# zhuye98/ICL

Measured on AMD Instinct MI355X. Metric: 3D volumes/sec/node (fwd+bwd, 96^3 patch), higher is better.
Workload: dtype f32; 1 GPU; 3D U-Net ICL BraTS-shape synthetic 96x96x96, num_classes=2, batch=2 per GPU (1 labeled + 1 unlabeled), full ICL step incl. SGD; global_batch=2, parallelism=dp1, launch=hipGraph replay

## Files before the change

### icl_amd/_lib.py

```python
from __future__ import annotations

import ctypes
import os
from ctypes import c_char_p, c_double, c_float, c_int, c_int64, c_void_p

import torch

_HERE = os.path.dirname(os.path.abspath(__file__))
DEFAULT_LIB = os.path.join(_HERE, "libicl_hip.so")

_lib = None
_lib_path = None
_host_pointers_ok = False

P, I, L, F = c_void_p, c_int, c_int64, c_float
D = c_double

_SIGNATURES = {
    "icl_abi_version": (c_int, []),
    "icl_last_error": (c_char_p, []),
    "icl_last_kernel_name": (c_char_p, []),
    "icl_conv3d_packed_elems": (c_int64, [I, I, I, I]),
    "icl_conv3d_pack_weights": (c_int, [P, P, I, I, I, I, P]),
    "icl_conv3d_pack_weights_both": (c_int, [P, P, P, I, I, I, P]),
# ... 2 lines not shown
    "icl_conv3d_fwd": (c_int, [P, P, P, P, P, I, I, I, I, I, I, I, L, L, P]),
    "icl_scalar_combine": (c_int, [P, P, I, I, P, P]),
    "icl_conv3d_split_ws_bytes": (c_int64, [I, I]),
    "icl_conv3d_split_weights_multi": (c_int, [P, P, P, P, I, P]),
    "icl_conv3d_fwd_presplit": (c_int, [P, P, P, P, I, I, I, I, I, I, L, L, P]),
    "icl_conv3d_fwd_presplit_ws_bytes": (c_int64, [I, I, I, I, I, I]),
    "icl_conv3d_fwd_presplit_ws": (c_int, [P, P, P, P, P, I, I, I, I, I, I, L, L, P]),
    "icl_conv3d_fwd_stats_slots": (c_int, [I, I, I, I, I, I]),
    "icl_conv3d_fwd_presplit_stats": (c_int, [P, P, P, P, P, I, I, I, I, I, I, L, L, P]),
    "icl_norm_fwd_given_stats": (c_int, [P, P, P, P, P, P, P, P, P, I, I, L, I, I, F, F, P, I, P]),
    "icl_conv3d_wgrad_ws_bytes": (c_int64, [I, I, I, I]),
    "icl_conv3d_wgrad": (c_int, [P, P, P, P, P, I, I, I, I, I, I, I, L, L, P]),
    "icl_conv3d_wgrad_slabs": (c_int, [P, P, P, I, I, I, I, I, I, I, L, L, P, P]),
    "icl_conv3d_wgrad_reduce_multi": (c_int, [P, P, P, P, P, P, I, P]),
    "icl_norm_ws_bytes": (c_int64, [I, I, L]),
    "icl_norm_fwd": (c_int, [P, P, P, P, P, P, P, P, I, I, L, I, I, I, F, F, P, P]),
    "icl_norm_bwd": (c_int, [P, P, P, P, P, P, P, P, P, I, I, L, I, I, I, P, P]),
    "icl_norm_res_fwd": (c_int, [P, P, P, P, P, P, P, P, P, I, I, L, I, I, I, F, F, P, P]),
    "icl_norm_res_bwd": (c_int, [P, P, P, P, P, P, P, P, P, P, P, I, I, L, I, I, I, P, P]),
    "icl_rstd_from_var": (c_int, [P, P, I, F, P]),
    "icl_norm_finalize_stats": (c_int, [P, I, I, I, F, P, P, P, P]),
    "icl_norm_apply": (c_int, [P, P, P, I, I, L, P]),
    "icl_maxpool2_fwd_norm": (c_int, [P, P, P, P, L, I, I, I, I, P]),
    "icl_upsample2x_concat_norm": (c_int, [P, P, P, P, P, I, I, I, I, I, I, P]),
    "icl_conv1x1_dropout_norm": (c_int, [P, P, P, P, P, I, I, I, L, I, I, ctypes.c_uint32, F, P, P]),
    "icl_conv1x1_wgrad_dropout_norm": (c_int, [P, P, P, P, P, P, I, I, I, L, L, ctypes.c_uint32, F, P, P]),
    "icl_maxpool2_fwd": (c_int, [P, P, P, L, I, I, I, I, P]),
    "icl_maxpool2_bwd": (c_int, [P, P, P, L, I, I, I, I, P]),
    "icl_maxpool2_bwd_add": (c_int, [P, P, P, P, I, I, I, I, I, I, L, P]),
    "icl_trilinear_fwd": (c_int, [P, P, I, I, I, I, I, I, I, I, L, I, P]),
    "icl_trilinear_bwd_ws_bytes": (c_int64, [I, I, I, I, I, I, I, I]),
    "icl_trilinear_bwd": (c_int, [P, P, P, I, I, I, I, I, I, I, I, L, I, P]),
    "icl_copy_rows": (c_int, [P, P, L, L, L, L, P]),
    "icl_concat2": (c_int, [P, L, P, L, P, P]),
    "icl_dwconv3_fwd": (c_int, [P, P, P, I, I, I, I, I, I, P]),
    "icl_dwconv3_wgrad_ws_bytes": (c_int64, [I, I, I, I, I]),
    "icl_dwconv3_wgrad": (c_int, [P, P, P, P, I, I, I, I, I, P]),
    "icl_conv1x1_small": (c_int, [P, P, P, P, I, I, I, L, I, I, P]),
    "icl_conv1x1_dropout": (c_int, [P, P, P, P, I, I, I, L, I, I, I, ctypes.c_uint32, F, P, P]),
    "icl_conv1x1_wgrad_dropout": (c_int, [P, P, P, P, P, I, I, I, L, L, ctypes.c_uint32, F, P, P]),
    "icl_dropout": (c_int, [P, P, L, ctypes.c_uint32, F, P, P]),
    "icl_drop_path": (c_int, [P, P, L, L, ctypes.c_uint32, F, P, P]),
    "icl_drop_path_add": (c_int, [P, P, P, L, L, ctypes.c_uint32, F, P, P]),
    "icl_loss_fwd": (c_int, [P, P, P, P, P, P, I, I, L, I, I, P]),
    "icl_window_attn_bias_elems": (c_int64, [I, I]),
    "icl_depth_to_space2": (c_int, [P, P, I, I, I, I, I, L, P]),
    "icl_space_to_depth2": (c_int, [P, P, I, I, I, I, I, L, P]),
    "icl_colsum_multi": (c_int, [P, P, P, P, I, P]),
    "icl_gather_rows": (c_int, [P, P, P, L, L, L, I, P]),
    "icl_gather_rows_sum2": (c_int, [P, P, P, L, L, L, I, P]),
    "icl_im2col3": (c_int, [P, P, I, I, I, I, I, P]),
    "icl_im2col3_planes": (c_int, [P, P, I, I, I, I, I, P]),
    "icl_conv3d_cin1_fwd": (c_int, [P, P, P, P, I, I, I, I, I, L, L, P]),
    "icl_conv3d_cin1_wgrad_ws_bytes": (c_int64, [I, I, I]),
    "icl_conv3d_cin1_wgrad": (c_int, [P, P, P, P, I, I, I, I, I, L, L, P]),
    "icl_col2im3": (c_int, [P, P, I, I, I, I, I, P]),
    "icl_linear_ws_bytes": (c_int64, [L, I, I, I]),
    "icl_linear_fwd": (c_int, [P, P, P, P, P, L, I, I, I, P]),
    "icl_linear_dgrad": (c_int, [P, P, P, P, L, I, I, P]),
    "icl_linear_bwd_small": (c_int, [P, P, P, P, P, P, L, I, I, P]),
    "icl_linear_wgrad_small": (c_int, [P, P, P, P, L, I, I, P]),
    "icl_linear_dgrad_sgd": (c_int, [P, P, P, P, P, P, L, I, I, F, F, F, I, P, P]),
    "icl_gemm_ws_bytes": (c_int64, [L, I, I, I]),
    "icl_gemm": (c_int, [P, P, P, P, P, L, I, I, L, L, L, I, I, I, I, L, L, L, P]),
    "icl_linear_wgrad_ws_bytes": (c_int64, [L, I, I]),
    "icl_linear_wgrad": (c_int, [P, P, P, P, P, L, I, I, P]),
    "icl_conv1x1_wgrad_ws_bytes": (c_int64, [I, L, I, I]),
    "icl_conv1x1_wgrad": (c_int, [P, P, P, P, P, I, I, I, L, L, L, P]),
    "icl_relpos_bias_fwd": (c_int, [P, P, P, I, I, I, P]),
    "icl_window_attn_fwd": (c_int, [P, P, P, P, P, I, I, I, I, I, F, P]),
    "icl_window_attn_bwd": (c_int, [P, P, P, P, P, P, P, P, I, I, I, I, I, F, P]),
    "icl_window_attn_bwd_chunks": (c_int, [I, I, I, I, I]),
    "icl_window_attn_fwd_drop": (c_int, [P, P, P, P, P, I, I, I, I, I, F, ctypes.c_uint32, F, P, P]),
    "icl_window_attn_keep_probe": (c_int, [P, c_int64, I, ctypes.c_uint32, F, P, P]),
    "icl_window_attn_bwd_drop": (c_int, [P, P, P, P, P, P, P, P, I, I, I, I, I, F, ctypes.c_uint32, F, P, P]),
    "icl_relpos_bias_bwd_sum": (c_int, [P, I, P, P, P, L, I, I, P]),
    "icl_layernorm_fwd": (c_int, [P, P, P, P, P, P, L, I, F, P]),
    "icl_layernorm_bwd_ws_bytes": (c_int64, [L, I]),
    "icl_layernorm_bwd": (c_int, [P, P, P, P, P, P, P, P, P, L, I, P]),
    "icl_gelu_fwd": (c_int, [P, P, L, P]),
    "icl_gelu_bwd": (c_int, [P, P, P, L, P]),
    "icl_attn_fwd": (c_int, [P, P, P, P, P, I, I, I, I, I, F, P]),
    "icl_attn_bwd": (c_int, [P, P, P, P, P, P, P, P, P, I, I, I, I, I, F, P]),
    "icl_attn_bwd_ws_bytes": (c_int64, [I, I, I, I, I]),
    "icl_attn_bwd_ws": (c_int, [P, P, P, P, P, P, P, P, P, P, I, I, I, I, I, F, P]),
    "icl_crop_rotflip": (c_int, [P, P, P, I, P, P, I, I, I, P]),
    "icl_volume_feed": (c_int, [P, P, P, P, I, P, P, I, I, I, P]),
    "icl_slice_augment": (c_int, [P, P, P, P, I, P, P, I, I, P]),
    "icl_slice_resize": (c_int, [P, P, L, I, I, I, I, I, P]),
    "icl_sgd_step": (c_int, [P, P, P, L, F, F, F, I, P, P]),
    "icl_sgd_step_factored": (c_int, [P, P, P, P, I, I, I, F, F, F, I, P, P]),
    "icl_sgd_step_factored_narrow": (c_int, [P, P, P, P, I, I, I, F, F, F, I, P, I, P]),
    "icl_sgd_factored_split_ws_bytes": (c_int64, [I, I, I]),
    "icl_sgd_step_factored_split": (c_int, [P, P, P, P, P, I, I, I, F, F, F, I, P, P]),
    "icl_sgd_step_multi": (c_int, [P, P, P, P, I, F, F, F, I, P, P]),
    "icl_loss_bwd": (c_int, [P, P, P, P, P, P, P, P, I, I, L, I, I, P]),
    "icl_loss_fwd_multi": (c_int, [P, I, P]),
    "icl_loss_bwd_multi": (c_int, [P, I, P]),
    "icl_qchain_stage": (c_int, [P, P]),
    "icl_qchain_wgrad": (c_int, [P, P, P, P, P, P, P, P, I, P]),
    "icl_seg_metrics_ws_bytes": (c_int64, [I, I, I, I]),
    "icl_seg_metrics": (c_int, [P, I, P, I, I, I, I, I, I, P, P, P]),
    "icl_seg_surface_ws_bytes": (c_int64, [I, I, I, I]),
    "icl_seg_surface_metrics": (c_int, [P, I, P, I, I, I, I, I, D, D, D, D, P, P, P, P]),
    "icl_window_gather": (c_int, [P, P, P, I, I, I, I, I, I, I, I, I, I, I, I, I, I, P]),
    "icl_window_accumulate": (c_int, [P, P, P, P, P, I, I, I, I, I, I, I, I, I, P]),
# ... 49 lines not shown
```

### icl_amd/csrc/icl_abi.inc

```

#include "kernels/common.h"
#include "kernels/norm.h"
#include "kernels/pool_resize.h"
#include "kernels/reduce.h"
#include "kernels/conv_mfma.h"
#include "kernels/conv_mfma_static.h"
#include "kernels/conv_mfma_flat.h"
#include "kernels/conv_bf16x3.h"
#include "kernels/conv_bf16x3_ws.h"
#include "kernels/conv_wgrad_tr.h"
#include "kernels/conv_wgrad_zs.h"
#include "kernels/conv_cin1.h"
#include "kernels/misc.h"
#include "kernels/loss.h"
#include "kernels/optim.h"
#include "kernels/winattn.h"
#include "kernels/linear_wgrad.h"
#include "kernels/token.h"
#include "kernels/gemm.h"
#include "kernels/datafeed.h"
#include "kernels/qchain.h"
#include "kernels/metrics.h"
#include "kernels/metrics_surface.h"
#include "kernels/window.h"
// ... 1815 lines not shown
  } else {
    if (tiled) ICL_LAUNCH((icl::attn_bwd_kv_kernel<8, true>), g1, dim3(256), 0, st, q, kv, logits, stats, out, gout, glog, gkv, b, h, nc, n, scale, pq);
    else ICL_LAUNCH((icl::attn_bwd_kv_kernel<8, false>), g1, dim3(256), 0, st, q, kv, logits, stats, out, gout, glog, gkv, b, h, nc, n, scale, pq);
    if (!pq) ICL_LAUNCH((icl::attn_bwd_q_kernel<8, 256>), g2, dim3(256), 0, st, kv, logits, stats, out, gout, glog, gq, b, h, nc, n, scale);
  }
  if (pq) {
    const int rd = b * h * nc * d;
    ICL_LAUNCH(icl::attn_dq_reduce_kernel, dim3((rd + 255) / 256), dim3(256), 0, st, (const float*)pq, gq, (int)g1.x, rd, scale);
  }
  return check_launch("attn_bwd");
}

int64_t icl_window_attn_bias_elems(int n, int heads) { return icl_window_attn_bias_elems_impl(n, heads); }

static int linear_wgrad_nsplit(int64_t rows, int o, int i) {
  const int ob = (o + icl::kLwB - 1) / icl::kLwB, ib = (i + icl::kLwB - 1) / icl::kLwB;
  long n = rows * (o + i) / ((long)o * i + o);
  const long want = (2048 + ob * ib - 1) / (ob * ib);
  if (n > want) n = want;
  const long steps = (rows + 3) / 4;
  if (n > steps / 8) n = steps / 8;
  if (n < 4) n = 4;
  return (int)((n + 3) / 4 * 4);
}

int64_t icl_linear_wgrad_ws_bytes(int64_t rows, int o, int i) {
  return (int64_t)linear_wgrad_nsplit(rows, o, i) * ((int64_t)o * i + o) * 4;
}

int icl_linear_wgrad(const float* gy, const float* x, float* dw, float* db, void* ws, int64_t rows, int o, int i, void* stream) {
  if (!gy || !x || !dw || !ws || rows < 1 || o < 1 || i < 1) return fail(-1, "linear_wgrad: bad argument");
  hipStream_t st = (hipStream_t)stream;
  const int nsplit = linear_wgrad_nsplit(rows, o, i);
  const int ob = (o + icl::kLwB - 1) / icl::kLwB, ib = (i + icl::kLwB - 1) / icl::kLwB;
  ICL_LAUNCH(icl::linear_wgrad_kernel, dim3(nsplit / 4, ob, ib), dim3(256), 0, st, gy, x, (float*)ws, (long)rows, o, i, nsplit);
  if (int rc = check_launch("linear_wgrad")) return rc;
  const long EW = (long)o * i, E = EW + o;
  ICL_LAUNCH(icl::linear_wgrad_reduce_kernel, dim3((unsigned)cdivl(E, 16)), dim3(256), 0, st, (const float*)ws, dw, db, E, EW, nsplit);
  return check_launch("linear_wgrad_reduce");
}

static bool cin1_geom(icl::Cin1Geom& g, int n, int cout, int d, int h, int w, int64_t xbs, int64_t ybs) {
  if (n < 1 || cout < 1 || cout > 16 || d < 1 || h < 1 || w < 1 || (long)d * h * w * 16 >= (1L << 31)) return false;
  g.N = n; g.Cout = cout; g.D = d; g.H = h; g.W = w; g.nty = (h + icl::kC1Rows - 1) / icl::kC1Rows;
  g.x_bstride = xbs; g.y_bstride = ybs; g.ntiles = n * d * g.nty;
  return (size_t)3 * (icl::kC1Rows + 2) * (w + 2) * 4 <= 64 * 1024;
}
static int cin1_grid(const icl::Cin1Geom& g) { return g.ntiles < 2048 ? g.ntiles : 2048; }
static size_t cin1_lds(const icl::Cin1Geom& g) {
  const size_t halo = (size_t)3 * (icl::kC1Rows + 2) * (g.W + 2) * 4;
  return halo > 2048 * 4 ? halo : 2048 * 4;
}

int icl_conv3d_cin1_fwd(const float* x, const float* w, const float* bias, float* y, int n, int cout, int d, int h, int wd, int64_t x_bstride,
                        int64_t y_bstride, void* stream) {
  icl::Cin1Geom g;
  if (!x || !w || !y || !cin1_geom(g, n, cout, d, h, wd, x_bstride, y_bstride)) return fail(-1, "conv3d_cin1_fwd: bad argument");
  ICL_LAUNCH(icl::conv_cin1_fwd_kernel, dim3(cin1_grid(g)), dim3(icl::kC1Threads), cin1_lds(g), (hipStream_t)stream, x, w, bias, y, g);
  snprintf(g_kernel, sizeof(g_kernel), "conv_cin1_fwd_kernel");
  return check_launch("conv3d_cin1_fwd");
}

int64_t icl_conv3d_cin1_wgrad_ws_bytes(int n, int d, int h) {
  const long tiles = (long)n * d * ((h + icl::kC1Rows - 1) / icl::kC1Rows);
  return (tiles < 2048 ? tiles : 2048) * 512 * 4;
}

int icl_conv3d_cin1_wgrad(const float* x, const float* gy, float* gw, void* ws, int n, int cout, int d, int h, int wd, int64_t x_bstride,
                          int64_t gy_bstride, void* stream) {
  icl::Cin1Geom g;
  if (!x || !gy || !gw || !ws || (wd & 3) || (gy_bstride & 3) || !aligned16(gy) || !cin1_geom(g, n, cout, d, h, wd, x_bstride, gy_bstride))
    return fail(-1, "conv3d_cin1_wgrad: bad argument (W and the sample stride of dY must be multiples of 4, dY 16-byte aligned)");
  const int grid = cin1_grid(g);
  ICL_LAUNCH(icl::conv_cin1_wgrad_kernel, dim3(grid), dim3(icl::kC1Threads), cin1_lds(g), (hipStream_t)stream, x, gy, (float*)ws, g);
  if (int rc = check_launch("conv3d_cin1_wgrad")) return rc;
  ICL_LAUNCH(icl::conv_cin1_wgrad_reduce_kernel, dim3(16), dim3(256), 0, (hipStream_t)stream, (const float*)ws, gw, grid, cout);
  snprintf(g_kernel, sizeof(g_kernel), "conv_cin1_wgrad_kernel");
  return check_launch("conv3d_cin1_wgrad_reduce");
}

int64_t icl_conv1x1_wgrad_ws_bytes(int n, int64_t s, int cin, int cout) { return icl_linear_wgrad_ws_bytes((int64_t)n * s, cout, cin); }

namespace {
int conv1x1_wgrad_run(const float* x, const float* gy, float* gw, float* gbias, void* ws, int n, int cin, int cout, int64_t s,
                      int64_t x_bstride, int64_t gy_bstride, const icl::DropSpec& dr, hipStream_t st) {
  const int nsplit = linear_wgrad_nsplit((int64_t)n * s, cout, cin);
  const int ob = (cout + icl::kLwB - 1) / icl::kLwB, ib = (cin + icl::kLwB - 1) / icl::kLwB;
  ICL_LAUNCH(icl::conv1x1_wgrad_kernel, dim3(nsplit / 4, ob, ib), dim3(256), 0, st, gy, x, (float*)ws, n, (long)s, cout, cin, nsplit,
             (long)gy_bstride, (long)x_bstride, dr);
  if (int rc = check_launch("conv1x1_wgrad")) return rc;
  const long EW = (long)cout * cin, E = EW + cout;
  ICL_LAUNCH(icl::linear_wgrad_reduce_kernel, dim3((unsigned)cdivl(E, 16)), dim3(256), 0, st, (const float*)ws, gw, gbias, E, EW, nsplit);
  return check_launch("conv1x1_wgrad_reduce");
}
}

int icl_conv1x1_wgrad(const float* x, const float* gy, float* gw, float* gbias, void* ws, int n, int cin, int cout, int64_t s,
                      int64_t x_bstride, int64_t gy_bstride, void* stream) {
  if (!x || !gy || !gw || !ws || n < 1 || cin < 1 || cout < 1 || s < 4 || (s & 3) || (x_bstride & 3) || (gy_bstride & 3))
    return fail(-1, "conv1x1_wgrad: bad argument (voxel count and batch strides must be multiples of 4)");
  return conv1x1_wgrad_run(x, gy, gw, gbias, ws, n, cin, cout, s, x_bstride, gy_bstride, icl::DropSpec{}, (hipStream_t)stream);
}

int icl_conv1x1_wgrad_dropout(const float* x, const float* gy, float* gw, float* gbias, void* ws, int n, int cin, int cout, int64_t s,
                              int64_t gy_bstride, uint32_t seed, float p, const uint32_t* seed_dev, void* stream) {
  if (!x || !gy || !gw || !ws || n < 1 || cin < 1 || cout < 1 || s < 4 || (s & 3) || (gy_bstride & 3) || !(p >= 0.f && p < 1.f))
    return fail(-1, "conv1x1_wgrad_dropout: bad argument");
  return conv1x1_wgrad_run(x, gy, gw, gbias, ws, n, cin, cout, s, (int64_t)cin * s, gy_bstride, drop_spec(1, seed, p, seed_dev), (hipStream_t)stream);
}

int icl_conv1x1_wgrad_dropout_norm(const float* x, const float* ss, const float* gy, float* gw, float* gbias, void* ws, int n, int cin, int cout,
                                   int64_t s, int64_t gy_bstride, uint32_t seed, float p, const uint32_t* seed_dev, void* stream) {
  if (!x || !ss || !gy || !gw || !ws || n < 1 || cin < 1 || cout < 1 || s < 4 || (s & 3) || (gy_bstride & 3) || !(p >= 0.f && p < 1.f))
    return fail(-1, "conv1x1_wgrad_dropout_norm: bad argument");
  icl::DropSpec dr = p > 0.f ? drop_spec(1, seed, p, seed_dev) : icl::DropSpec{};
  dr.ss = ss;
  return conv1x1_wgrad_run(x, gy, gw, gbias, ws, n, cin, cout, s, (int64_t)cin * s, gy_bstride, dr, (hipStream_t)stream);
}

int icl_relpos_bias_fwd(const float* table, const int64_t* index, float* bias, int n, int heads, int idx_stride, void* stream) {
  if (!table || !index || !bias || n < 1 || n > idx_stride || heads < 1) return fail(-1, "relpos_bias_fwd: bad argument");
  const int npad = (n + 15) / 16 * 16;
  ICL_LAUNCH(icl::relpos_bias_gather_kernel, dim3(grid_for((long)heads * n * npad, 256)), dim3(256), 0, (hipStream_t)stream, table,
             (const long*)index, bias, n, npad, heads, idx_stride);
  return check_launch("relpos_bias_fwd");
}

// ... 742 lines not shown
```

### icl_amd/csrc/kernels/conv_cin1.h

```cpp
#pragma once

namespace icl {

constexpr int kC1Rows = 8, kC1Threads = 256;

struct Cin1Geom {
  int N, Cout, D, H, W, nty;
  long x_bstride, y_bstride;
  int ntiles;
};

__device__ __forceinline__ void c1_stage_halo(float* xs, const float* __restrict__ x, const Cin1Geom& g, int n, int z, int y0) {
  const int PW = g.W + 2, PR = kC1Rows + 2;
  const long HW = (long)g.H * g.W;
  const float* xb = x + (long)n * g.x_bstride;
  for (int it = threadIdx.x; it < 3 * PR * PW; it += kC1Threads) {
    const int px = it % PW, row = it / PW, py = row % PR, pz = row / PR;
    const int gz = z - 1 + pz, gy = y0 - 1 + py, gx = px - 1;
    float v = 0.f;
    if ((unsigned)gz < (unsigned)g.D && (unsigned)gy < (unsigned)g.H && (unsigned)gx < (unsigned)g.W) v = xb[gz * HW + (long)gy * g.W + gx];
    xs[it] = v;
  }
}

// ... 72 lines not shown
  if (slice == 0) {
    float t = 0.f;
#pragma unroll
    for (int k = 0; k < 8; ++k) t += sl[k][o];
    const int co = e >> 5, tap = e & 31;
    if (co < cout && tap < 27) gw[co * 27 + tap] = t;
  }
}

__global__ __launch_bounds__(kC1Threads) void conv_cin1_fwd_kernel(const float* __restrict__ x, const float* __restrict__ w,
                                                                   const float* __restrict__ bias, float* __restrict__ y, Cin1Geom g) {
  ICL_DYN_LDS(float, xs);
  const int lane = threadIdx.x & 63, wid = threadIdx.x >> 6, lr = lane & 15, lg = lane >> 4;
  const int PW = g.W + 2, PR = kC1Rows + 2;
  const long HW = (long)g.H * g.W, DHW = g.D * HW;
  float wa[7];
  int toff[7];
#pragma unroll
  for (int s = 0; s < 7; ++s) {
    const int tap = 4 * s + lg;
    wa[s] = (tap < 27 && lr < g.Cout) ? w[lr * 27 + tap] : 0.f;
    const int t = tap < 27 ? tap : 0;
    toff[s] = (t / 9) * PR * PW + ((t / 3) % 3) * PW + t % 3;
  }
  float bv[4];
#pragma unroll
  for (int r = 0; r < 4; ++r) bv[r] = (bias && 4 * lg + r < g.Cout) ? bias[4 * lg + r] : 0.f;
  for (int tile = blockIdx.x; tile < g.ntiles; tile += gridDim.x) {
    const int n = tile / (g.D * g.nty), rem = tile % (g.D * g.nty), z = rem / g.nty, y0 = (rem % g.nty) * kC1Rows;
    __syncthreads();
    c1_stage_halo(xs, x, g, n, z, y0);
    __syncthreads();
    float* yb = y + (long)n * g.y_bstride + (long)z * HW;
    for (int rr = 0; rr < 2; ++rr) {
      const int ty = 2 * wid + rr, yy = y0 + ty;
      if (yy >= g.H) break;
      const float* xrow = xs + ty * PW;
      for (int x0 = 0; x0 < g.W; x0 += 16) {
        const int xp = x0 + lr;
        const bool in = xp < g.W;
        f32x4 acc = f32x4{bv[0], bv[1], bv[2], bv[3]};
#pragma unroll
        for (int s = 0; s < 7; ++s) acc = icl_mfma_16x16x4(wa[s], in ? xrow[toff[s] + xp] : 0.f, acc);
        if (in) {
#pragma unroll
          for (int r = 0; r < 4; ++r)
            if (4 * lg + r < g.Cout) yb[(long)(4 * lg + r) * DHW + (long)yy * g.W + xp] = acc[r];
        }
      }
    }
  }
}

}
```

### icl_amd/ops.py

```python
from __future__ import annotations

import ctypes
import math
import os
from typing import Optional, Sequence

import torch

from . import _lib
from .step_scope import BackwardEnd, DeferredBiasGrads, DeferredWgradReduce, FactoredGrads, ScopeField, StepScope, WgradLane

_vp = ctypes.c_void_p


def _ptr(t: Optional[torch.Tensor]):
    return None if t is None else _vp(t.data_ptr())


def _stream(t: torch.Tensor):
    if t.is_cuda:
        return _vp(torch.cuda.current_stream(t.device).cuda_stream)
    return None


# ... 304 lines not shown
        z = _ZERO_CACHE[key] = torch.zeros(n, dtype=torch.float32, device=device)
    return z


CONV1X1_WGRAD_MIN_VOXELS = 4096
FIRST_CONV_PLANES_MAX_K = 32
CONV1X1_GEMM_MIN_VOXELS = 65536
CONV1X1_SMALL_MAX_CHANNELS = 16


class _Conv3d(torch.autograd.Function):
    @staticmethod
    def forward(ctx, x, weight, bias, zero_bias_grad=False, want_stats=False):
        y = _Conv3d._forward(ctx, x, weight, bias, zero_bias_grad, want_stats)
        if not want_stats:
            return y
        ctx.set_materialize_grads(False)
        stats = ctx.stats if getattr(ctx, "stats", None) is not None else torch.empty(0, dtype=torch.float32, device=x.device)
        ctx.stats = None
        ctx.mark_non_differentiable(stats)
        return y, stats

    @staticmethod
    def _forward(ctx, x, weight, bias, zero_bias_grad, want_stats):
        _require(x, weight, bias)
        x = x.contiguous()
        weight = weight.contiguous()
        ctx.zero_bias_grad = zero_bias_grad
        n, cin, d, h, w = x.shape
        cout, ks = weight.shape[0], weight.shape[2]
        assert weight.shape[1] == cin and weight.shape[2] == weight.shape[3] == weight.shape[4]
        s = d * h * w
        ctx.save_for_backward(x, weight)
        if ks == 3:
            WgradLane.note_use(weight)
        ctx.has_bias = bias is not None
        small_ch = cin <= CONV1X1_SMALL_MAX_CHANNELS and cout <= CONV1X1_SMALL_MAX_CHANNELS and s % 4 == 0
        ctx.pointwise_gemm = ks == 1 and n * s >= CONV1X1_GEMM_MIN_VOXELS and not small_ch
        if ctx.pointwise_gemm:
            y = torch.empty((n, cout, d, h, w), dtype=torch.float32, device=x.device)
            gemm(weight, x, cout, s, cin, cin, s, True, False, out=y, ldc=s, bias=bias, act=16, batch=n, b_bstride=cin * s,
                 c_bstride=cout * s)
            return y
        y = torch.empty((n, cout, d, h, w), dtype=torch.float32, device=x.device)
        ctx.wpt = None
        ctx.pointwise_small = ks == 1 and small_ch
        if ctx.pointwise_small:
            _lib.check(_lib.lib().icl_conv1x1_small(_ptr(x), _ptr(weight), _ptr(bias), _ptr(y), n, cin, cout, s, cin, 1, _stream(x)),
                       "conv1x1_small")
            return y
        ctx.cin1 = (ks == 3 and cin == 1 and cout <= 16 and not ctx.needs_input_grad[0] and 120 * (w + 2) <= 65536
                    and os.environ.get("ICL_CONV_CIN1", "1") != "0")
        if ctx.cin1:
            with _timed("conv_cin1_fwd_kernel", 2.0 * 27 * cout * s * n, 4.0 * n * s * (1 + cout), x):
                _lib.check(_lib.lib().icl_conv3d_cin1_fwd(_ptr(x), _ptr(weight), _ptr(bias), _ptr(y), n, cout, d, h, w, cin * s, cout * s,
                                                          _stream(x)), "conv3d_cin1_fwd")
            return y
        wsf = ctx.wsd = None
        if ctx.needs_input_grad[0]:
            wp, ctx.wpt = PackedWeights.get(weight)
            wsf, ctx.wsd = PackedWeights.split_of(weight)
            if ks == 3:
                PackedWeights.note_volume(weight, s)
        else:
            wp = pack_weights(weight, 0)
        ctx.stats = conv3d_forward_raw(x, wp, bias, n, cin, cout, d, h, w, ks, cin * s, y, cout * s, wsplit=wsf, want_stats=want_stats)
        return y

    @staticmethod
    def backward(ctx, gy, gstats=None):
        if gy is None:
            return None, None, None, None, None
        x, weight = ctx.saved_tensors
        L = _lib.lib()
        gy = gy.contiguous()
        n, cin, d, h, w = x.shape
        cout, ks = weight.shape[0], weight.shape[2]
        s = d * h * w
        gx = gw = gb = None
        lane = (ks == 3 and WgradLane.wants(x, s) and ctx.needs_input_grad[0] and ctx.needs_input_grad[1] and not getattr(ctx, "cin1", False)
                and not (cin * 27 <= FIRST_CONV_PLANES_MAX_K))
        if lane:
            WgradLane.fork_point(gy)
        if ctx.needs_input_grad[0]:
            if ctx.pointwise_gemm:
                gx = torch.empty_like(x)
                gemm(weight, gy, cin, s, cout, cin, s, False, False, out=gx, ldc=s, batch=n, b_bstride=cout * s, c_bstride=cin * s)
            elif ctx.pointwise_small:
                gx = torch.empty_like(x)
                _lib.check(L.icl_conv1x1_small(_ptr(gy), _ptr(weight), None, _ptr(gx), n, cout, cin, s, 1, cin, _stream(x)),
                           "conv1x1_small dgrad")
            else:
                gx = torch.empty_like(x)
                wpt = ctx.wpt if ctx.wpt is not None else pack_weights(weight, 1)
                conv3d_forward_raw(gy, wpt, None, n, cout, cin, d, h, w, ks, cout * s, gx, cin * s, wsplit=getattr(ctx, "wsd", None))
        if ctx.needs_input_grad[1] or (ctx.has_bias and ctx.needs_input_grad[2]):
            gw = torch.empty_like(weight)
            gb = torch.empty(cout, dtype=torch.float32, device=x.device) if ctx.has_bias else None
            gb_arg = gb
            if ctx.has_bias and ctx.zero_bias_grad:
                gb = _cached_zeros(cout, x.device).view(cout) if getattr(StepScope.current, "packed", None) is not None else x.new_zeros(cout)
                gb_arg = None
            flops = 2.0 * ks ** 3 * cin * cout * s * n
            nbytes = 4.0 * (n * s * (cin + cout) + 2 * ks ** 3 * cin * cout)
            if ks == 1 and s % 4 == 0 and n * s >= CONV1X1_WGRAD_MIN_VOXELS:
                ws = _ws(L.icl_conv1x1_wgrad_ws_bytes(n, s, cin, cout), x)
                with _timed("conv1x1_wgrad_kernel", flops, nbytes, x):
# ... 1948 lines not shown
```

### include/icl_hip.h

```cpp
#ifndef ICL_HIP_H
#define ICL_HIP_H
#include <stdint.h>
#ifdef __cplusplus
extern "C" {
#endif

int icl_abi_version(void);
const char* icl_last_error(void);
const char* icl_last_kernel_name(void);

int64_t icl_conv3d_packed_elems(int cout, int cin, int ks, int mode);
int icl_conv3d_pack_weights(const float* w, float* wp, int cout, int cin, int ks, int mode, void* stream);
int icl_conv3d_pack_weights_both(const float* w, float* wp_fwd, float* wp_dgrad, int cout, int cin, int ks, void* stream);
int icl_conv3d_pack_weights_multi(const void* const* w, void* const* wp_fwd, void* const* wp_dgrad, const int32_t* cout, const int32_t* cin,
                                  const int32_t* ks, int count, void* stream);
int64_t icl_conv3d_fwd_ws_bytes(int n, int cin, int cout, int d, int h, int w, int ks);
int64_t icl_conv3d_split_ws_bytes(int cin, int cout);
int icl_conv3d_split_weights_multi(const void* const* wp, void* const* wsplit, const int32_t* cin, const int32_t* cout, int count,
                                   void* stream);
int icl_conv3d_fwd_presplit(const float* x, const void* wsplit, const float* bias, float* y, int n, int cin, int cout, int d, int h, int w,
                            int64_t x_bstride, int64_t y_bstride, void* stream);
int64_t icl_conv3d_fwd_presplit_ws_bytes(int n, int cin, int cout, int d, int h, int w);
int icl_conv3d_fwd_presplit_ws(const float* x, const void* wsplit, const float* bias, float* y, void* ws, int n, int cin, int cout, int d,
                               int h, int w, int64_t x_bstride, int64_t y_bstride, void* stream);
// ... 64 lines not shown
int icl_conv1x1_dropout_norm(const float* x, const float* ss, const float* w, const float* bias, float* y, int n, int cin, int cout, int64_t s,
                             int w_ostride, int w_istride, uint32_t seed, float p, const uint32_t* seed_dev, void* stream);
int icl_conv1x1_wgrad_dropout_norm(const float* x, const float* ss, const float* gy, float* gw, float* gbias, void* ws, int n, int cin,
                                   int cout, int64_t s, int64_t gy_bstride, uint32_t seed, float p, const uint32_t* seed_dev, void* stream);

int icl_dropout(const float* x, float* y, int64_t n, uint32_t seed, float p, const uint32_t* seed_dev, void* stream);
int icl_drop_path(const float* x, float* y, int64_t n, int64_t group, uint32_t seed, float p, const uint32_t* seed_dev, void* stream);
int icl_drop_path_add(const float* x, const float* res, float* y, int64_t n, int64_t group, uint32_t seed, float p,
                      const uint32_t* seed_dev, void* stream);

#define ICL_LOSS_MAX_BLOCKS 1024
#define ICL_LOSS_STATS_FLOATS(nc) ((3 * (nc) + 1) * (1 + ICL_LOSS_MAX_BLOCKS))
int icl_loss_fwd(const float* a, const float* b, const int64_t* labels, const float* weight, float* stats, float* out,
                 int batch, int nc, int64_t s, int mode, int a_is_prob, void* stream);
int icl_loss_bwd(const float* a, const float* b, const int64_t* labels, const float* weight, const float* stats,
                 const float* gout0, const float* gout1, float* ga, int batch, int nc, int64_t s, int mode, int a_is_prob,
                 void* stream);
typedef struct IclLossJob {
  const float* a; const float* b; const int64_t* labels; const float* weight;
  float* stats; float* out;
  const float* gout0; const float* gout1; float* ga;
  int64_t s;
  int batch, nc, mode, a_is_prob;
} IclLossJob;
int icl_loss_fwd_multi(const IclLossJob* jobs, int count, void* stream);
int icl_loss_bwd_multi(const IclLossJob* jobs, int count, void* stream);

int icl_layernorm_fwd(const float* x, const float* gamma, const float* beta, float* y, float* mean, float* rstd, int64_t rows,
                      int c, float eps, void* stream);
int64_t icl_layernorm_bwd_ws_bytes(int64_t rows, int c);
int icl_layernorm_bwd(const float* gy, const float* x, const float* gamma, const float* mean, const float* rstd, float* gx,
                      float* dgamma, float* dbeta, void* ws, int64_t rows, int c, void* stream);
int icl_gelu_fwd(const float* x, float* y, int64_t n, void* stream);
int icl_gelu_bwd(const float* gy, const float* x, float* gx, int64_t n, void* stream);
int icl_attn_fwd(const float* q, const float* kv, float* logits, float* out, float* stats, int b, int h, int nc, int n, int d,
                 float scale, void* stream);
int icl_attn_bwd(const float* q, const float* kv, const float* logits, const float* stats, const float* out, const float* gout,
                 const float* glog, float* gq, float* gkv, int b, int h, int nc, int n, int d, float scale, void* stream);
int64_t icl_attn_bwd_ws_bytes(int b, int h, int nc, int n, int d);
int icl_attn_bwd_ws(const float* q, const float* kv, const float* logits, const float* stats, const float* out, const float* gout,
                    const float* glog, float* gq, float* gkv, void* ws, int b, int h, int nc, int n, int d, float scale, void* stream);

int icl_colsum_multi(const void* const* g, void* const* out, const int32_t* rows, const int32_t* cols, int count, void* stream);
int icl_scalar_combine(const void* const* in, const float* w, int n_in, int n_out, float* out, void* stream);

int icl_gather_rows(const float* src, const int32_t* idx, float* out, int64_t b, int64_t s, int64_t m, int c, void* stream);
int icl_gather_rows_sum2(const float* src, const int32_t* idx2, float* out, int64_t b, int64_t s, int64_t m, int c, void* stream);

int icl_im2col3(const float* x, float* cols, int n, int c, int d, int h, int w, void* stream);
int icl_im2col3_planes(const float* x, float* planes, int n, int c, int d, int h, int w, void* stream);

int icl_conv3d_cin1_fwd(const float* x, const float* w, const float* bias, float* y, int n, int cout, int d, int h, int wd, int64_t x_bstride,
                        int64_t y_bstride, void* stream);
int64_t icl_conv3d_cin1_wgrad_ws_bytes(int n, int d, int h);
int icl_conv3d_cin1_wgrad(const float* x, const float* gy, float* gw, void* ws, int n, int cout, int d, int h, int wd, int64_t x_bstride,
                          int64_t gy_bstride, void* stream);
int icl_col2im3(const float* g, float* dx, int n, int c, int d, int h, int w, void* stream);

int icl_depth_to_space2(const float* yt, float* out, int n, int d, int h, int w, int cout, int64_t out_bstride, void* stream);
int icl_space_to_depth2(const float* g, float* gt, int n, int d, int h, int w, int cout, int64_t g_bstride, void* stream);

int64_t icl_linear_ws_bytes(int64_t rows, int in, int out, int kind);
int icl_linear_fwd(const float* x, const float* w, const float* bias, float* y, void* ws, int64_t rows, int in, int out, int act,
                   void* stream);
int icl_linear_dgrad(const float* gy, const float* w, float* gx, void* ws, int64_t rows, int in, int out, void* stream);
int icl_linear_bwd_small(const float* gy, const float* w, const float* x, float* gx, float* dw, void* ws, int64_t rows, int in, int out,
                         void* stream);
int icl_linear_wgrad_small(const float* gy, const float* x, float* dw, void* ws, int64_t rows, int in, int out, void* stream);
int icl_linear_dgrad_sgd(const float* gy, const float* x, float* w, float* mom, float* gx, void* ws, int64_t rows, int in, int out,
                         float lr, float momentum, float weight_decay, int first, const float* lr_dev, void* stream);
int64_t icl_gemm_ws_bytes(int64_t m, int n, int k, int batch);
int icl_gemm(const float* a, const float* b, float* c, const float* bias, void* ws, int64_t m, int n, int k, int64_t lda, int64_t ldb,
             int64_t ldc, int a_kcontig, int b_kcontig, int act, int batch, int64_t a_bstride, int64_t b_bstride, int64_t c_bstride,
             void* stream);

int64_t icl_linear_wgrad_ws_bytes(int64_t rows, int o, int i);
int icl_linear_wgrad(const float* gy, const float* x, float* dw, float* db, void* ws, int64_t rows, int o, int i, void* stream);

int64_t icl_conv1x1_wgrad_ws_bytes(int n, int64_t s, int cin, int cout);
int icl_conv1x1_wgrad(const float* x, const float* gy, float* gw, float* gbias, void* ws, int n, int cin, int cout, int64_t s,
                      int64_t x_bstride, int64_t gy_bstride, void* stream);

int64_t icl_window_attn_bias_elems(int n, int heads);
int icl_relpos_bias_fwd(const float* table, const int64_t* index, float* bias, int n, int heads, int idx_stride, void* stream);
int icl_window_attn_fwd(const float* qkv, const float* bias, const int32_t* regions, float* out, float* lse, int b_, int n, int heads,
                        int nw, int head_dim, float scale, void* stream);
int icl_window_attn_bwd(const float* qkv, const float* bias, const int32_t* regions, const float* out, const float* lse,
                        const float* dout, float* dqkv, float* dbias, int b_, int n, int heads, int nw, int head_dim, float scale,
                        void* stream);
int icl_window_attn_fwd_drop(const float* qkv, const float* bias, const int32_t* regions, float* out, float* lse, int b_, int n, int heads,
                             int nw, int head_dim, float scale, uint32_t seed, float p, const uint32_t* seed_dev, void* stream);
int icl_window_attn_bwd_drop(const float* qkv, const float* bias, const int32_t* regions, const float* out, const float* lse,
                             const float* dout, float* dqkv, float* dbias, int b_, int n, int heads, int nw, int head_dim, float scale,
                             uint32_t seed, float p, const uint32_t* seed_dev, void* stream);
int icl_window_attn_keep_probe(int32_t* out, int64_t base, int count, uint32_t seed, float p, const uint32_t* seed_dev, void* stream);
int icl_window_attn_bwd_chunks(int b_, int n, int heads, int nw, int head_dim);
int icl_relpos_bias_bwd_sum(float* dbias, int chunks, const int32_t* inv, const int32_t* offs, float* dtable, int64_t table_rows, int n,
                            int heads, void* stream);

int icl_crop_rotflip(const void* const* images, const void* const* labels, const int32_t* params, int batch, float* image_out,
                     int64_t* label_out, int o0, int o1, int o2, void* stream);

int icl_volume_feed(const void* const* images, const void* const* labels, const int32_t* int_params, const float* float_params, int batch,
                    float* image_out, int64_t* label_out, int R0, int R1, int R2, void* stream);

int icl_slice_augment(const void* const* images, const void* const* labels, const int32_t* int_params, const double* double_params,
// ... 50 lines not shown
```

Baseline: 204.5 volumes/s.

## Add z-walking ring-buffer kernels for Cin=1 conv fwd/wgrad with fused norm stats

Adds forward and weight-grad kernels for the first (single input channel) 3D conv. Each workgroup walks a run of z planes and keeps a 4-slot LDS ring of halo planes, so every input plane is loaded once instead of being re-staged per tile. The next plane is prefetched into registers while the current one is computed. The forward kernel can also emit per-slot mean/M2 partial statistics, so the following normalization does not need a separate pass over the output. The wgrad kernel prefetches dY in chunks and writes bounded partials. The cost is more template variants, more register pressure, and double-precision stats accumulation.

```diff
diff --git a/icl_amd/_lib.py b/icl_amd/_lib.py
--- a/icl_amd/_lib.py
+++ b/icl_amd/_lib.py
@@ -78,6 +78,8 @@
     "icl_im2col3": (c_int, [P, P, I, I, I, I, I, P]),
     "icl_im2col3_planes": (c_int, [P, P, I, I, I, I, I, P]),
     "icl_conv3d_cin1_fwd": (c_int, [P, P, P, P, I, I, I, I, I, L, L, P]),
+    "icl_conv3d_cin1_fwd_stats_slots": (c_int, [I, I, I, I, I]),
+    "icl_conv3d_cin1_fwd_stats": (c_int, [P, P, P, P, P, I, I, I, I, I, L, L, P]),
     "icl_conv3d_cin1_wgrad_ws_bytes": (c_int64, [I, I, I]),
     "icl_conv3d_cin1_wgrad": (c_int, [P, P, P, P, I, I, I, I, I, L, L, P]),
     "icl_col2im3": (c_int, [P, P, I, I, I, I, I, P]),
diff --git a/icl_amd/csrc/icl_abi.inc b/icl_amd/csrc/icl_abi.inc
--- a/icl_amd/csrc/icl_abi.inc
+++ b/icl_amd/csrc/icl_abi.inc
@@ -1891,13 +1891,84 @@
   return halo > 2048 * 4 ? halo : 2048 * 4;
 }
 
+static int cin1_walk_nl(const icl::Cin1Geom& g, bool wgrad = false) {
+  const char* e = getenv("ICL_CIN1_WALK");
+  if (e && (atoi(e) == 0 || (wgrad && atoi(e) == 2))) return 0;
+  const int plane = (icl::kC1Rows + 2) * (g.W + 2);
+  if ((size_t)icl::kC1Slots * plane * 4 > (size_t)kMaxDynLds) return 0;
+  const int nl = (plane + icl::kC1Threads - 1) / icl::kC1Threads;
+  return nl <= 4 ? 4 : nl <= 8 ? 8 : nl <= 16 ? 16 : 0;
+}
+static size_t cin1_walk_lds(const icl::Cin1Geom& g) {
+  const size_t ring = (size_t)icl::kC1Slots * (icl::kC1Rows + 2) * (g.W + 2) * 4;
+  return ring > 2048 * 4 ? ring : 2048 * 4;
+}
+static icl::Cin1Walk cin1_walk_plan(const icl::Cin1Geom& g, int want) {
+  icl::Cin1Walk wk{};
+  const int cols = g.N * g.nty;
+  const char* e = getenv("ICL_CIN1_ZRUN");
+  int zrun = e ? atoi(e) : 0;
+  if (zrun < 1) {
+    int rpc = want / cols;
+    rpc = rpc < 1 ? 1 : (rpc > g.D ? g.D : rpc);
+    zrun = (g.D + rpc - 1) / rpc;
+  }
+  if (zrun > g.D) zrun = g.D;
+  wk.zrun = zrun;
+  wk.nruns = (g.D + zrun - 1) / zrun;
+  wk.total = cols * wk.nruns;
+  wk.slots = g.nty * wk.nruns;
+  return wk;
+}
+constexpr int kC1FwdWgs = 576, kC1WgradWgs = 384, kC1MaxParts = 512;
+
+extern "C++" {
+template <int NL>
+static void cin1_fwd_walk_launch(const float* x, const float* w, const float* bias, float* y, float* stats, const icl::Cin1Geom& g,
+                                 const icl::Cin1Walk& wk, hipStream_t st) {
+  ICL_LAUNCH((icl::conv_cin1_fwd_walk_kernel<NL>), dim3(wk.total), dim3(icl::kC1Threads), cin1_walk_lds(g), st, x, w, bias, y, stats, g, wk);
+}
+template <int NL>
+static void cin1_wgrad_walk_launch(const float* x, const float* gy, float* part, int grid, const icl::Cin1Geom& g, const icl::Cin1Walk& wk,
+                                   hipStream_t st) {
+  ICL_LAUNCH((icl::conv_cin1_wgrad_walk_kernel<NL>), dim3(grid), dim3(icl::kC1Threads), cin1_walk_lds(g), st, x, gy, part, g, wk);
+}
+}
+
+static int cin1_fwd(const float* x, const float* w, const float* bias, float* y, float* stats, int n, int cout, int d, int h, int wd,
+                    int64_t x_bstride, int64_t y_bstride, void* stream) {
+  icl::Cin1Geom g;
+  if (!x || !w || !y || !cin1_geom(g, n, cout, d, h, wd, x_bstride, y_bstride)) return fail(-1, "conv3d_cin1_fwd: bad argument");
+  const int nl = cin1_walk_nl(g);
+  if (stats && !nl) return fail(-1, "conv3d_cin1_fwd_stats: this shape hands out no statistics (icl_conv3d_cin1_fwd_stats_slots)");
+  if (nl) {
+    icl::Cin1Walk wk = cin1_walk_plan(g, kC1FwdWgs);
+    wk.vec = (wd & 3) == 0 && (y_bstride & 3) == 0 && aligned16(y);
+    if (nl == 4) cin1_fwd_walk_launch<4>(x, w, bias, y, stats, g, wk, (hipStream_t)stream);
+    else if (nl == 8) cin1_fwd_walk_launch<8>(x, w, bias, y, stats, g, wk, (hipStream_t)stream);
+    else cin1_fwd_walk_launch<16>(x, w, bias, y, stats, g, wk, (hipStream_t)stream);
+  } else {
+    ICL_LAUNCH(icl::conv_cin1_fwd_kernel, dim3(cin1_grid(g)), dim3(icl::kC1Threads), cin1_lds(g), (hipStream_t)stream, x, w, bias, y, g);
+  }
+  snprintf(g_kernel, sizeof(g_kernel), "conv_cin1_fwd_kernel");
+  return check_launch("conv3d_cin1_fwd");
+}
+
 int icl_conv3d_cin1_fwd(const float* x, const float* w, const float* bias, float* y, int n, int cout, int d, int h, int wd, int64_t x_bstride,
                         int64_t y_bstride, void* stream) {
+  return cin1_fwd(x, w, bias, y, nullptr, n, cout, d, h, wd, x_bstride, y_bstride, stream);
+}
+
+int icl_conv3d_cin1_fwd_stats_slots(int n, int cout, int d, int h, int wd) {
   icl::Cin1Geom g;
-  if (!x || !w || !y || !cin1_geom(g, n, cout, d, h, wd, x_bstride, y_bstride)) return fail(-1, "conv3d_cin1_fwd: bad argument");
-  ICL_LAUNCH(icl::conv_cin1_fwd_kernel, dim3(cin1_grid(g)), dim3(icl::kC1Threads), cin1_lds(g), (hipStream_t)stream, x, w, bias, y, g);
-  snprintf(g_kernel, sizeof(g_kernel), "conv_cin1_fwd_kernel");
-  return check_launch("conv3d_cin1_fwd");
+  if (!cin1_geom(g, n, cout, d, h, wd, (int64_t)d * h * wd, (int64_t)cout * d * h * wd) || !cin1_walk_nl(g)) return 0;
+  return cin1_walk_plan(g, kC1FwdWgs).slots;
+}
+
+int icl_conv3d_cin1_fwd_stats(const float* x, const float* w, const float* bias, float* y, float* stats, int n, int cout, int d, int h, int wd,
+                              int64_t x_bstride, int64_t y_bstride, void* stream) {
+  if (!stats) return fail(-1, "conv3d_cin1_fwd_stats: bad argument");
+  return cin1_fwd(x, w, bias, y, stats, n, cout, d, h, wd, x_bstride, y_bstride, stream);
 }
 
 int64_t icl_conv3d_cin1_wgrad_ws_bytes(int n, int d, int h) {
@@ -1910,8 +1981,17 @@
   icl::Cin1Geom g;
   if (!x || !gy || !gw || !ws || (wd & 3) || (gy_bstride & 3) || !aligned16(gy) || !cin1_geom(g, n, cout, d, h, wd, x_bstride, gy_bstride))
     return fail(-1, "conv3d_cin1_wgrad: bad argument (W and the sample stride of dY must be multiples of 4, dY 16-byte aligned)");
-  const int grid = cin1_grid(g);
-  ICL_LAUNCH(icl::conv_cin1_wgrad_kernel, dim3(grid), dim3(icl::kC1Threads), cin1_lds(g), (hipStream_t)stream, x, gy, (float*)ws, g);
+  int grid;
+  if (const int nl = cin1_walk_nl(g, true)) {
+    const icl::Cin1Walk wk = cin1_walk_plan(g, kC1WgradWgs);
+    grid = wk.total < kC1MaxParts ? wk.total : kC1MaxParts;
+    if (nl == 4) cin1_wgrad_walk_launch<4>(x, gy, (float*)ws, grid, g, wk, (hipStream_t)stream);
+    else if (nl == 8) cin1_wgrad_walk_launch<8>(x, gy, (float*)ws, grid, g, wk, (hipStream_t)stream);
+    else cin1_wgrad_walk_launch<16>(x, gy, (float*)ws, grid, g, wk, (hipStream_t)stream);
+  } else {
+    grid = cin1_grid(g);
+    ICL_LAUNCH(icl::conv_cin1_wgrad_kernel, dim3(grid), dim3(icl::kC1Threads), cin1_lds(g), (hipStream_t)stream, x, gy, (float*)ws, g);
+  }
   if (int rc = check_launch("conv3d_cin1_wgrad")) return rc;
   ICL_LAUNCH(icl::conv_cin1_wgrad_reduce_kernel, dim3(16), dim3(256), 0, (hipStream_t)stream, (const float*)ws, gw, grid, cout);
   snprintf(g_kernel, sizeof(g_kernel), "conv_cin1_wgrad_kernel");
diff --git a/icl_amd/csrc/kernels/conv_cin1.h b/icl_amd/csrc/kernels/conv_cin1.h
--- a/icl_amd/csrc/kernels/conv_cin1.h
+++ b/icl_amd/csrc/kernels/conv_cin1.h
@@ -148,4 +148,270 @@
   }
 }
 
-}
+constexpr int kC1Slots = 4;
+constexpr int kC1PF = 12;
+
+struct Cin1Walk {
+  int zrun, nruns, total;
+  int vec;
+  int slots;
+};
+
+template <int NL>
+__device__ __forceinline__ void c1_plane_items(int (&off)[NL], const Cin1Geom& g, int y0) {
+  const int PW = g.W + 2, PR = kC1Rows + 2;
+#pragma unroll
+  for (int k = 0; k < NL; ++k) {
+    const int it = threadIdx.x + kC1Threads * k, py = it / PW, px = it - py * PW;
+    const int gy = y0 - 1 + py, gx = px - 1;
+    off[k] = (py < PR && (unsigned)gy < (unsigned)g.H && (unsigned)gx < (unsigned)g.W) ? gy * g.W + gx : -1;
+  }
+}
+template <int NL>
+__device__ __forceinline__ void c1_plane_load(float (&r)[NL], const int (&off)[NL], const float* __restrict__ xb, const Cin1Geom& g, int z) {
+  const bool zin = (unsigned)z < (unsigned)g.D;
+  const float* xz = xb + (long)(zin ? z : 0) * g.H * g.W;
+#pragma unroll
+  for (int k = 0; k < NL; ++k) r[k] = (zin && off[k] >= 0) ? xz[off[k]] : 0.f;
+}
+template <int NL>
+__device__ __forceinline__ void c1_plane_deposit(const float (&r)[NL], float* slot, int plane) {
+#pragma unroll
+  for (int k = 0; k < NL; ++k) {
+    const int it = threadIdx.x + kC1Threads * k;
+    if (it < plane) slot[it] = r[k];
+  }
+}
+template <int NL>
+__device__ __forceinline__ void c1_stage_extra(float* xs, const int (&off)[NL], const float* __restrict__ xb, const Cin1Geom& g, int z0, int plane) {
+  float r0[NL], r1[NL], r2[NL];
+  c1_plane_load(r0, off, xb, g, z0 - 1);
+  c1_plane_load(r1, off, xb, g, z0);
+  c1_plane_load(r2, off, xb, g, z0 + 1);
+  c1_plane_deposit(r0, xs, plane);
+  c1_plane_deposit(r1, xs + plane, plane);
+  c1_plane_deposit(r2, xs + 2 * plane, plane);
+}
+
+struct C1Sums {
+  double n, s, ss;
+};
+__device__ __forceinline__ void c1_stats_add(C1Sums& run, const float* v, const int* cnt) {
+#pragma unroll
+  for (int i = 0; i < 16; ++i)
+    if ((i & 3) < cnt[i >> 2]) {
+      const double d = (double)v[i];
+      run.s += d;
+      run.ss = fma(d, d, run.ss);
+      run.n += 1.0;
+    }
+}
+__device__ __forceinline__ void c1_stats_flush(const C1Sums& run, double* scratch, float* out, int cout, int slots, int slot) {
+  double* mine = scratch + 3 * threadIdx.x;
+  mine[0] = run.n; mine[1] = run.s; mine[2] = run.ss;
+  __syncthreads();
+  if (threadIdx.x < 16 && (int)threadIdx.x < cout) {
+    double n = 0.0, s = 0.0, ss = 0.0;
+    for (int t = threadIdx.x; t < kC1Threads; t += 16) {
+      n += scratch[3 * t]; s += scratch[3 * t + 1]; ss += scratch[3 * t + 2];
+    }
+    double mean = 0.0, m2 = 0.0;
+    if (n > 0.0) {
+      mean = s / n;
+      m2 = ss - s * mean;
+      if (m2 < 0.0) m2 = 0.0;
+    }
+    float* o = out + ((long)threadIdx.x * slots + slot) * 3;
+    o[0] = (float)n; o[1] = (float)mean; o[2] = (float)m2;
+  }
+}
+
+template <int NL>
+__global__ __launch_bounds__(kC1Threads) void conv_cin1_fwd_walk_kernel(const float* __restrict__ x, const float* __restrict__ w,
+                                                                        const float* __restrict__ bias, float* __restrict__ y,
+                                                                        float* __restrict__ stats, Cin1Geom g, Cin1Walk wk) {
+  ICL_DYN_LDS(float, xs);
+  const int lane = threadIdx.x & 63, wid = threadIdx.x >> 6, lr = lane & 15, lg = lane >> 4;
+  const int PW = g.W + 2, PLANE = (kC1Rows + 2) * PW;
+  const long HW = (long)g.H * g.W, DHW = g.D * HW;
+  float wb[7];
+  int tdz[7], tin[7];
+#pragma unroll
+  for (int s = 0; s < 7; ++s) {
+    const int tap = 4 * s + lg;
+    wb[s] = (tap < 27 && lr < g.Cout) ? w[lr * 27 + tap] : 0.f;
+    const int t = tap < 27 ? tap : 0;
+    tdz[s] = t / 9;
+    tin[s] = ((t / 3) % 3) * PW + t % 3;
+  }
+  const float bv = (bias && lr < g.Cout) ? bias[lr] : 0.f;
+  const int col = blockIdx.x / wk.nruns, rz = blockIdx.x - col * wk.nruns, n = col / g.nty, band = col - n * g.nty;
+  const int y0 = band * kC1Rows, z0 = rz * wk.zrun, z1 = z0 + wk.zrun < g.D ? z0 + wk.zrun : g.D;
+  const float* xb = x + (long)n * g.x_bstride;
+  float* yb = y + (long)n * g.y_bstride + (long)lr * DHW;
+  int off[NL];
+  c1_plane_items(off, g, y0);
+  c1_stage_extra(xs, off, xb, g, z0, PLANE);
+  __syncthreads();
+  const int gpr = (g.W + 15) >> 4;
+  int nrow = g.H - (y0 + 2 * wid);
+  nrow = nrow < 0 ? 0 : (nrow > 2 ? 2 : nrow);
+  const int ng = nrow * gpr;
+  C1Sums run = {0.0, 0.0, 0.0};
+  int rb = 0;
+  for (int z = z0; z < z1; ++z) {
+    const bool more = z + 1 < z1;
+    float nx[NL];
+    if (more) c1_plane_load(nx, off, xb, g, z + 2);
+    int toff[7];
+#pragma unroll
+    for (int s = 0; s < 7; ++s) toff[s] = ((rb + tdz[s]) & 3) * PLANE + tin[s];
+    for (int c0 = 0; c0 < ng; c0 += 4) {
+      float sv[16];
+      int scnt[4];
+#pragma unroll
+      for (int j = 0; j < 4; ++j) {
+        const int gi = c0 + j;
+        scnt[j] = 0;
+#pragma unroll
+        for (int r = 0; r < 4; ++r) sv[4 * j + r] = 0.f;
+        if (gi < ng) {
+          const int rr = gi >= gpr ? 1 : 0, x0 = (gi - rr * gpr) << 4, ty = 2 * wid + rr, yy = y0 + ty;
+          const int xp = x0 + lr;
+          const bool in = xp < g.W;
+          const float* xrow = xs + ty * PW + xp;
+          f32x4 acc = f32x4{bv, bv, bv, bv};
+#pragma unroll
+          for (int s = 0; s < 7; ++s) acc = icl_mfma_16x16x4(in ? xrow[toff[s]] : 0.f, wb[s], acc);
+          const int xq = x0 + 4 * lg;
+          float* yp = yb + (long)z * HW + (long)yy * g.W + xq;
+          if (lr < g.Cout) {
+            if (wk.vec) {
+              if (xq < g.W) *reinterpret_cast<float4*>(yp) = make_float4(acc[0], acc[1], acc[2], acc[3]);
+            } else {
+#pragma unroll
+              for (int r = 0; r < 4; ++r)
+                if (xq + r < g.W) yp[r] = acc[r];
+            }
+          }
+#pragma unroll
+          for (int r = 0; r < 4; ++r) sv[4 * j + r] = acc[r];
+          scnt[j] = g.W - xq < 0 ? 0 : (g.W - xq > 4 ? 4 : g.W - xq);
+        }
+      }
+      if (stats) c1_stats_add(run, sv, scnt);
+    }
+    if (more) c1_plane_deposit(nx, xs + ((rb + 3) & 3) * PLANE, PLANE);
+    __syncthreads();
+    rb = (rb + 1) & 3;
+  }
+  if (stats)
+    c1_stats_flush(run, reinterpret_cast<double*>(xs), stats + (long)n * g.Cout * wk.slots * 3, g.Cout, wk.slots, band * wk.nruns + rz);
+}
+
+template <int NL>
+__global__ __launch_bounds__(kC1Threads) void conv_cin1_wgrad_walk_kernel(const float* __restrict__ x, const float* __restrict__ gy,
+                                                                          float* __restrict__ part, Cin1Geom g, Cin1Walk wk) {
+  ICL_DYN_LDS(float, xs);
+  const int lane = threadIdx.x & 63, wid = threadIdx.x >> 6, lr = lane & 15, lg = lane >> 4;
+  const int PW = g.W + 2, PLANE = (kC1Rows + 2) * PW;
+  const long HW = (long)g.H * g.W, DHW = g.D * HW;
+  int tdz[2], tin[2];
+  bool tok[2];
+#pragma unroll
+  for (int tb = 0; tb < 2; ++tb) {
+    const int tap = 16 * tb + lr;
+    tok[tb] = tap < 27;
+    const int t = tok[tb] ? tap : 0;
+    tdz[tb] = t / 9;
+    tin[tb] = ((t / 3) % 3) * PW + t % 3;
+  }
+  const int gpr = (g.W + 15) >> 4;
+  f32x4 acc[2] = {f32x4{0.f, 0.f, 0.f, 0.f}, f32x4{0.f, 0.f, 0.f, 0.f}};
+  for (int run = blockIdx.x; run < wk.total; run += gridDim.x) {
+    const int col = run / wk.nruns, rz = run - col * wk.nruns, n = col / g.nty, y0 = (col - n * g.nty) * kC1Rows;
+    const int z0 = rz * wk.zrun, z1 = z0 + wk.zrun < g.D ? z0 + wk.zrun : g.D;
+    const float* xb = x + (long)n * g.x_bstride;
+    const float* gb = gy + (long)n * g.y_bstride + (long)lr * DHW + (long)(y0 + 2 * wid) * g.W + 4 * lg;
+    int off[NL];
+    c1_plane_items(off, g, y0);
+    c1_stage_extra(xs, off, xb, g, z0, PLANE);
+    __syncthreads();
+    int nrow = g.H - (y0 + 2 * wid);
+    nrow = nrow < 0 ? 0 : (nrow > 2 ? 2 : nrow);
+    const int ng = nrow * gpr, nchunk = (ng + kC1PF - 1) / kC1PF;
+    auto load_gy = [&](float4 (&dst)[kC1PF], int z, int p) {
+#pragma unroll
+      for (int j = 0; j < kC1PF; ++j) {
+        const int gi = p * kC1PF + j;
+        dst[j] = make_float4(0.f, 0.f, 0.f, 0.f);
+        if (gi < ng) {
+          const int rr = gi >= gpr ? 1 : 0, x0 = (gi - rr * gpr) << 4;
+          if (lr < g.Cout && x0 + 4 * lg < g.W) dst[j] = *reinterpret_cast<const float4*>(gb + (long)z * HW + rr * g.W + x0);
+        }
+      }
+    };
+    float4 cur[kC1PF], nxt[kC1PF];
+    if (nchunk) load_gy(cur, z0, 0);
+    int rb = 0;
+    for (int z = z0; z < z1; ++z) {
+      const bool more = z + 1 < z1;
+      float nx[NL];
+      if (more) c1_plane_load(nx, off, xb, g, z + 2);
+      int toff[2];
+#pragma unroll
+      for (int tb = 0; tb < 2; ++tb) toff[tb] = ((rb + tdz[tb]) & 3) * PLANE + tin[tb];
+      for (int p = 0; p < nchunk; ++p) {
+        const bool wrap = p + 1 == nchunk;
+        const int pn = wrap ? 0 : p + 1, zn = wrap ? z + 1 : z;
+        const bool have = zn < z1;
+        if (have) load_gy(nxt, zn, pn);
+#pragma unroll
+        for (int j = 0; j < kC1PF; ++j) {
+          const int gi = p * kC1PF + j;
+          if (gi < ng) {
+            const int rr = gi >= gpr ? 1 : 0, x0 = (gi - rr * gpr) << 4, xl = x0 + 4 * lg;
+            const bool in = xl < g.W;
+            const float* xrow = xs + (2 * wid + rr) * PW + xl;
+            const float av[4] = {cur[j].x, cur[j].y, cur[j].z, cur[j].w};
+#pragma unroll
+            for (int q = 0; q < 4; ++q) {
+#pragma unroll
+              for (int tb = 0; tb < 2; ++tb) {
+                const float b = (tok[tb] && in) ? xrow[toff[tb] + q] : 0.f;
+                acc[tb] = icl_mfma_16x16x4(av[q], b, acc[tb]);
+              }
+            }
+          }
+        }
+        if (have) {
+#pragma unroll
+          for (int j = 0; j < kC1PF; ++j) cur[j] = nxt[j];
+        }
+      }
+      if (more) c1_plane_deposit(nx, xs + ((rb + 3) & 3) * PLANE, PLANE);
+      __syncthreads();
+      rb = (rb + 1) & 3;
+    }
+  }
+  __syncthreads();
+  float* red = xs;
+#pragma unroll
+  for (int tb = 0; tb < 2; ++tb)
+#pragma unroll
+    for (int r = 0; r < 4; ++r) red[((wid * 2 + tb) * 4 + r) * 64 + lane] = acc[tb][r];
+  __syncthreads();
+  if (wid == 0) {
+#pragma unroll
+    for (int tb = 0; tb < 2; ++tb)
+#pragma unroll
+      for (int r = 0; r < 4; ++r) {
+        float s = 0.f;
+#pragma unroll
+        for (int w = 0; w < 4; ++w) s += red[((w * 2 + tb) * 4 + r) * 64 + lane];
+        part[(long)blockIdx.x * 512 + (4 * lg + r) * 32 + 16 * tb + lr] = s;
+      }
+  }
+}
+
+}
diff --git a/icl_amd/ops.py b/icl_amd/ops.py
--- a/icl_amd/ops.py
+++ b/icl_amd/ops.py
@@ -380,7 +380,15 @@
         ctx.cin1 = (ks == 3 and cin == 1 and cout <= 16 and not ctx.needs_input_grad[0] and 120 * (w + 2) <= 65536
                     and os.environ.get("ICL_CONV_CIN1", "1") != "0")
         if ctx.cin1:
+            L = _lib.lib()
+            slots = (L.icl_conv3d_cin1_fwd_stats_slots(n, cout, d, h, w)
+                     if want_stats and os.environ.get("ICL_CONV_STATS", "1") != "0" else 0)
             with _timed("conv_cin1_fwd_kernel", 2.0 * 27 * cout * s * n, 4.0 * n * s * (1 + cout), x):
+                if slots > 0:
+                    ctx.stats = torch.empty((n * cout, slots, 3), dtype=torch.float32, device=x.device)
+                    _lib.check(L.icl_conv3d_cin1_fwd_stats(_ptr(x), _ptr(weight), _ptr(bias), _ptr(y), _ptr(ctx.stats), n, cout, d, h, w,
+                                                           cin * s, cout * s, _stream(x)), "conv3d_cin1_fwd_stats")
+                    return y
                 _lib.check(_lib.lib().icl_conv3d_cin1_fwd(_ptr(x), _ptr(weight), _ptr(bias), _ptr(y), n, cout, d, h, w, cin * s, cout * s,
                                                           _stream(x)), "conv3d_cin1_fwd")
             return y
diff --git a/include/icl_hip.h b/include/icl_hip.h
--- a/include/icl_hip.h
+++ b/include/icl_hip.h
@@ -140,6 +140,9 @@
 
 int icl_conv3d_cin1_fwd(const float* x, const float* w, const float* bias, float* y, int n, int cout, int d, int h, int wd, int64_t x_bstride,
                         int64_t y_bstride, void* stream);
+int icl_conv3d_cin1_fwd_stats_slots(int n, int cout, int d, int h, int wd);
+int icl_conv3d_cin1_fwd_stats(const float* x, const float* w, const float* bias, float* y, float* stats, int n, int cout, int d, int h, int wd,
+                              int64_t x_bstride, int64_t y_bstride, void* stream);
 int64_t icl_conv3d_cin1_wgrad_ws_bytes(int n, int d, int h);
 int icl_conv3d_cin1_wgrad(const float* x, const float* gy, float* gw, void* ws, int n, int cout, int d, int h, int wd, int64_t x_bstride,
                           int64_t gy_bstride, void* stream);
```

Result: no change. 204.3 volumes/s (-0.1%).
